# cvg/LightGlue

Measured on AMD Instinct MI355X. Metric: image-pairs/s at N=M=1024, 9 layers; match-index parity vs ref, higher is better.
Workload: dtype f16; 1 GPU; SuperPoint-dim 256-d descriptors, N=M=1024, 9 layers, pruning/early-stop OFF, batch=32 pairs per GPU, seeded random weights (recipe A), precision=f16x3 (split-f16 operands, 3 MFMAs per product, for every contraction incl. q k^T and P V; fp32 accumulate / residual / softmax); pairs_per_gpu=32, keypoints=1024, keypoints1=1024, descriptor_dim=256, parallelism=pair-sharded dp1, batches_in_flight=1

## Files before the change

lightglue_amd/csrc/lg_assign.hip:

```cpp
#include "lg_kernels.h"

namespace lg {

__device__ __forceinline__ float fexp(float x) { return __builtin_amdgcn_exp2f(x * 1.44269504088896340736f); }

__device__ __forceinline__ void lse_merge(float& m, float& s, float m2, float s2) {
    const float mn = fmaxf(m, m2);
    if (mn == -INFINITY) { m = mn; s = 0.f; return; }
    s = s * fexp(m - mn) + s2 * fexp(m2 - mn);
    m = mn;
}

constexpr int ART = 32;

__device__ __forceinline__ void lse_merge1(float& m, float& s, float m2, float s2) {
    const float e = (m == m2) ? 1.f : fexp(-fabsf(m - m2));
    const bool keep = m >= m2;
    s = keep ? __builtin_fmaf(s2, e, s) : __builtin_fmaf(s, e, s2);
    m = keep ? m : m2;
}

__global__ __launch_bounds__(256) void lse_sweep_kernel(AssignArgs a) {
    const int pair = blockIdx.y, tile = blockIdx.x, tid = threadIdx.x, lane = tid & 63, wave = tid >> 6;
    const int len0 = a.rs.len[2 * pair], len1 = a.rs.len[2 * pair + 1];
    const int r0 = tile * ART;
    if (r0 >= len0) return;
    const int rows = min(ART, len0 - r0);
    const int ntiles = a.rs.cap0 / ART;
    const float* simp = a.sim + ((long long)pair * a.rs.cap0 + r0) * a.rs.cap1;
    float* pm = a.cpm + ((long long)pair * ntiles + tile) * a.rs.cap1;
    float* ps = a.cps + ((long long)pair * ntiles + tile) * a.rs.cap1;
    __shared__ float shm[4][ART], shs[4][ART];
    for (int c0 = 0; c0 < len1; c0 += 1024) {
        const int c = c0 + tid * 4;
        const bool act = c < len1;
        const float* col = simp + (act ? c : 0);
        float cm[4] = {-INFINITY, -INFINITY, -INFINITY, -INFINITY}, cs[4] = {0.f, 0.f, 0.f, 0.f};
        f32x4 nxt = *reinterpret_cast<const f32x4*>(col);
#pragma unroll 1
        for (int r = 0; r < rows; ++r) {
            f32x4 v = nxt;
            nxt = *reinterpret_cast<const f32x4*>(col + (long long)min(r + 1, rows - 1) * a.rs.cap1);
#pragma unroll
            for (int i = 0; i < 4; ++i) if (!act || c + i >= len1) v[i] = -INFINITY;
            const float m = wave_allmax(fmaxf(fmaxf(v[0], v[1]), fmaxf(v[2], v[3])));
            float sum = 0.f;
            if (m != -INFINITY) sum = (fexp(v[0] - m) + fexp(v[1] - m)) + (fexp(v[2] - m) + fexp(v[3] - m));
            if (act) {
#pragma unroll
                for (int i = 0; i < 4; ++i) lse_merge1(cm[i], cs[i], v[i], v[i] == -INFINITY ? 0.f : 1.f);
            }
            sum = wave_allsum(sum);
            if (lane == 0) {
                if (c0 == 0) { shm[wave][r] = m; shs[wave][r] = sum; }
                else { float mo = shm[wave][r], so = shs[wave][r]; lse_merge1(mo, so, m, sum); shm[wave][r] = mo; shs[wave][r] = so; }
            }
        }
        if (act) {
            *reinterpret_cast<f32x4*>(pm + c) = f32x4{cm[0], cm[1], cm[2], cm[3]};
            *reinterpret_cast<f32x4*>(ps + c) = f32x4{cs[0], cs[1], cs[2], cs[3]};
        }
    }
    __syncthreads();
    if (tid < rows) {
        float m = shm[0][tid], s = shs[0][tid];
        for (int w = 1; w < 4; ++w) lse_merge1(m, s, shm[w][tid], shs[w][tid]);
        a.lse_r[(long long)pair * a.rs.cap0 + r0 + tid] = m + logf(s);
    }
}

__global__ __launch_bounds__(256) void col_lse_merge_kernel(AssignArgs a) {
    const int pair = blockIdx.y, lane = threadIdx.x & 63, wave = threadIdx.x >> 6, c = blockIdx.x * 64 + lane;
    const int len0 = a.rs.len[2 * pair], len1 = a.rs.len[2 * pair + 1];
    if (blockIdx.x * 64 >= len1) return;
    const int ntiles = a.rs.cap0 / ART, live = (len0 + ART - 1) / ART;
    const int cc = min(c, a.rs.cap1 - 1);
    const float* pm = a.cpm + (long long)pair * ntiles * a.rs.cap1 + cc;
    const float* ps = a.cps + (long long)pair * ntiles * a.rs.cap1 + cc;
    float m = -INFINITY, s = 0.f;
#pragma unroll 8
    for (int t = wave; t < live; t += 4) lse_merge1(m, s, pm[(long long)t * a.rs.cap1], ps[(long long)t * a.rs.cap1]);
    __shared__ float shm[4][64], shs[4][64];
    shm[wave][lane] = m; shs[wave][lane] = s;
    __syncthreads();
    if (wave == 0 && c < len1) {
#pragma unroll
        for (int w = 1; w < 4; ++w) lse_merge1(m, s, shm[w][lane], shs[w][lane]);
        a.lse_c[(long long)pair * a.rs.cap1 + c] = m + logf(s);
    }
}

__device__ __forceinline__ float score_of(float sim, float lr, float lc, float cert) {
    return ((sim - lr) + (sim - lc)) + cert;
}

__global__ __launch_bounds__(256) void argmax_sweep_kernel(AssignArgs a) {
    const int pair = blockIdx.y, tile = blockIdx.x, tid = threadIdx.x, lane = tid & 63, wave = tid >> 6;
    const int len0 = a.rs.len[2 * pair], len1 = a.rs.len[2 * pair + 1];
    const int r0 = tile * ART;
    if (r0 >= len0) return;
    const int rows = min(ART, len0 - r0);
    const int ntiles = a.rs.cap0 / ART;
    const float* simp = a.sim + ((long long)pair * a.rs.cap0 + r0) * a.rs.cap1;
    const float* lsec = a.lse_c + (long long)pair * a.rs.cap1;
    const float* ls1 = a.ls + seg_row_base(a.rs, 2 * pair + 1);
    const float* lser = a.lse_r + (long long)pair * a.rs.cap0 + r0;
    const float* ls0 = a.ls + seg_row_base(a.rs, 2 * pair) + r0;
    float* pv = a.cbv + ((long long)pair * ntiles + tile) * a.rs.cap1;
    int* pi = a.cbi + ((long long)pair * ntiles + tile) * a.rs.cap1;
    __shared__ float shb[4][ART]; __shared__ int shi[4][ART];
    for (int c0 = 0; c0 < len1; c0 += 1024) {
        const int c = c0 + tid * 4;
        const bool act = c < len1;
        const int cc = act ? c : 0;
        const float* col = simp + cc;
        const f32x4 lc = *reinterpret_cast<const f32x4*>(lsec + cc);
        const f32x4 l1 = *reinterpret_cast<const f32x4*>(ls1 + cc);
        float cb[4] = {-INFINITY, -INFINITY, -INFINITY, -INFINITY}; int ci[4] = {0, 0, 0, 0};
        f32x4 nxt = *reinterpret_cast<const f32x4*>(col);
#pragma unroll 1
        for (int r = 0; r < rows; ++r) {
// ... 133 lines not shown
    const int base0 = seg_row_base(a.rs, 2 * pair), base1 = seg_row_base(a.rs, 2 * pair + 1);
    float* out = a.log_assignment + (long long)pair * (a.n0 + 1) * (a.n1 + 1);
    if (len0 == 0 || len1 == 0) {
        if (r == a.rs.cap0 && tid == 0) out[(long long)a.n0 * (a.n1 + 1) + a.n1] = 0.f;
        return;
    }
    if (r == a.rs.cap0) {
        for (int c = tid; c < len1; c += 256) out[(long long)a.n0 * (a.n1 + 1) + a.ind[base1 + c]] = a.lsneg[base1 + c];
        if (tid == 0) out[(long long)a.n0 * (a.n1 + 1) + a.n1] = 0.f;
        return;
    }
    if (r >= len0) return;
    float* orow = out + (long long)a.ind[base0 + r] * (a.n1 + 1);
    const float* simr = a.sim + ((long long)pair * a.rs.cap0 + r) * a.rs.cap1;
    const float lr = a.lse_r[(long long)pair * a.rs.cap0 + r], l0 = a.ls[base0 + r];
    const float* lsec = a.lse_c + (long long)pair * a.rs.cap1;
    for (int c = tid; c < len1; c += 256) orow[a.ind[base1 + c]] = score_of(simr[c], lr, lsec[c], l0 + a.ls[base1 + c]);
    if (tid == 0) orow[a.n1] = a.lsneg[base0 + r];
}

hipError_t launch_assign(const AssignArgs& a, hipStream_t s) {
    const int B = a.rs.B;
    hipError_t e;
    if (!a.all_rows_live) {
    if (a.n0 > 0) {
        if ((e = hipMemsetAsync(a.m0, 0xFF, sizeof(int) * (size_t)B * a.n0, s)) != hipSuccess) return e;
        if ((e = hipMemsetAsync(a.s0, 0, sizeof(float) * (size_t)B * a.n0, s)) != hipSuccess) return e;
    }
    if (a.n1 > 0) {
        if ((e = hipMemsetAsync(a.m1, 0xFF, sizeof(int) * (size_t)B * a.n1, s)) != hipSuccess) return e;
        if ((e = hipMemsetAsync(a.s1, 0, sizeof(float) * (size_t)B * a.n1, s)) != hipSuccess) return e;
    }
    }
    hipLaunchKernelGGL(lse_sweep_kernel, dim3(a.rs.cap0 / ART, B), dim3(256), 0, s, a);
    hipLaunchKernelGGL(col_lse_merge_kernel, dim3(a.rs.cap1 / 64, B), dim3(256), 0, s, a);
    hipLaunchKernelGGL(argmax_sweep_kernel, dim3(a.rs.cap0 / ART, B), dim3(256), 0, s, a);
    hipLaunchKernelGGL(col_argmax_merge_kernel, dim3(a.rs.cap1 / 64, B), dim3(256), 0, s, a);
    hipLaunchKernelGGL(finalize_kernel, dim3((max(a.rs.cap0, a.rs.cap1) + 255) / 256, B), dim3(256), 0, s, a);
    if (a.log_assignment) {
        const long long total = (long long)B * (a.n0 + 1) * (a.n1 + 1);
        hipLaunchKernelGGL(fill_neg_inf_kernel, dim3(2048), dim3(256), 0, s, a.log_assignment, total);
        hipLaunchKernelGGL(log_assignment_kernel, dim3(a.rs.cap0 + 1, B), dim3(256), 0, s, a);
    }
    return hipGetLastError();
}

}
```

lightglue_amd/csrc/lg_engine.hip:

```cpp
#include <cmath>
#include <cstring>
#include <string>

#include "lg_engine.h"

using namespace lg;

namespace {

inline int round_up(int x, int m) { return (x + m - 1) / m * m; }
size_t attn_elem_bytes(int attn_prec) { return attn_prec == PREC_F32 ? 4 : attn_prec == PREC_F16X3 ? 4 : 2; }
int compact_chunks(int c0, int c1) { return (c0 > c1 ? c0 : c1) / compact_chunk_rows(); }
size_t cflags_bytes(int B, int c0, int c1) { return (size_t)2 * B * compact_chunks(c0, c1) * 4 + 256; }

}

namespace lg {

size_t workspace_layout(lg_engine* e, char* base, int B, int c0, int c1) {
    const size_t R = (size_t)B * (c0 + c1), as = attn_elem_bytes(e->attn_prec);
    const size_t per0 = (size_t)B * c0 * 4, per1 = (size_t)B * c1 * 4, tiles = (size_t)B * (c0 / 32) * c1 * 4;
    Arena ar{base};
    if (base) e->bufs.clear();
    auto take = [&](const char* name, auto*& member, size_t bytes) { ar.take(member, bytes); if (base) e->bufs[name] = {member, bytes}; };
// ... 60 lines not shown
void lg_engine_destroy(lg_engine* e) {
    if (!e) return;
    for (auto& sp : e->prof_pool) { (void)hipEventDestroy(sp.a); (void)hipEventDestroy(sp.b); }
    if (e->ws) (void)hipFree(e->ws);
    if (e->w_arena) (void)hipFree(e->w_arena);
    delete e;
}

static int check_envelope(long long B, long long n0, long long n1) {
    const long long c0 = (n0 + 127) / 128 * 128, c1 = (n1 + 127) / 128 * 128;
    if (n0 > LG_MAX_KEYPOINTS || n1 > LG_MAX_KEYPOINTS)
        return set_error(LG_ERR_INVALID, "more than LG_MAX_KEYPOINTS (8192) keypoints in one image");
    if (B * (c0 + c1) > LG_MAX_ROWS)
        return set_error(LG_ERR_INVALID, "batch * (cap0 + cap1) exceeds LG_MAX_ROWS (2^21 keypoint rows per forward): split the batch across calls");
    if (B * c0 * c1 > LG_MAX_SIM_ELEMS)
        return set_error(LG_ERR_INVALID, "batch * cap0 * cap1 exceeds LG_MAX_SIM_ELEMS (2^31 - 1 similarity entries per forward): split the batch across calls");
    return LG_OK;
}

int lg_engine_reserve(lg_engine* e, int32_t max_batch, int32_t max_n0, int32_t max_n1) {
    if (!e || max_batch < 1 || max_n0 < 0 || max_n1 < 0) return set_error(LG_ERR_INVALID, "bad argument");
    TRY(check_envelope(max_batch, max_n0, max_n1));
    return ensure_workspace(e, max_batch, max_n0, max_n1);
}

int lg_engine_set_option(lg_engine* e, const char* key, int32_t value) {
    if (!e || !key) return set_error(LG_ERR_INVALID, "null argument");
    if (std::strcmp(key, "fused_tail") == 0) { e->opt.fused_tail = value != 0; return LG_OK; }
    if (std::strcmp(key, "fused_next") == 0) { e->opt.fused_next = value != 0; return LG_OK; }
    if (std::strcmp(key, "fused_prep") == 0) { e->opt.fused_prep = value != 0; return LG_OK; }
    if (std::strcmp(key, "attn_dma") == 0) { e->opt.attn_dma = value != 0; return LG_OK; }
    if (std::strcmp(key, "adapt_gather") == 0) { e->opt.adapt_gather = value != 0; return LG_OK; }
    if (std::strcmp(key, "sim_planes") == 0) { e->opt.sim_planes = value != 0; return LG_OK; }
    if (std::strcmp(key, "sim_chunk") == 0) { if (value < 0 || value % 64) return set_error(LG_ERR_INVALID, "sim_chunk: 0 or a multiple of 64"); e->opt.sim_chunk = value; return LG_OK; }
    if (std::strcmp(key, "attn_rows") == 0) { if (value != 16 && value != 32 && value != 64) return set_error(LG_ERR_INVALID, "attn_rows must be 16, 32 or 64"); e->opt.attn_rows = value; e->opt.attn_auto_rows = false; return LG_OK; }
    if (std::strcmp(key, "tail_row_tiles") == 0) { if (value != 0 && value != 1 && value != 2 && value != 4) return set_error(LG_ERR_INVALID, "tail_row_tiles must be 0 (automatic), 1, 2 or 4"); e->opt.tail_row_tiles = value; return LG_OK; }
    if (std::strcmp(key, "profile_only") == 0) { e->prof_only = value; return LG_OK; }
    if (std::strcmp(key, "tail_timing") == 0) { e->opt.tail_timing = value; return LG_OK; }
    return set_error(LG_ERR_INVALID, std::string("unknown option '") + key + "'");
}

namespace {
int tail_row_tiles_for(int R) {
    int best = 4; long long best_cost = -1;
    const int shapes[3] = {4, 2, 1}; const long long cost[3] = {114, 69, 58};
    for (int i = 0; i < 3; ++i) {
        const long long wgs = R / (16 * shapes[i]), rounds = (wgs + 255) / 256, c = rounds * cost[i];
        if (best_cost < 0 || c < best_cost) { best = shapes[i]; best_cost = c; }
    }
    return best;
}

PairIndex pair_index(const lg_forward_io* io) { return indexed(io->flags) ? PairIndex{io->index0, io->index1, io->images0, io->images1} : PairIndex{}; }

int check_forward_io(const lg_engine* e, const lg_forward_io* io) {
    if (!e || !io) return set_error(LG_ERR_INVALID, "null argument");
    for (int side = 0; side < 2; ++side) {
        const SideFormat f = side_format(io->flags, side);
        if (!f.valid) return set_error(LG_ERR_INVALID, (io->flags & LG_FLAG_EXT) ? "LG_FLAG_DESC*_U8 and LG_FLAG_DESC*_F16 are both set on one side: a store has one format"
                                                                                 : "LG_FLAG_DESC*_F16 / LG_FLAG_DESC*_U8 / LG_FLAG_ROOTSIFT* need LG_FLAG_EXT");
        if (f.kind != DESC_F32 && (reinterpret_cast<uintptr_t>(side ? io->desc1 : io->desc0) & 15))
            return set_error(LG_ERR_INVALID, "LG_FLAG_DESC*_F16 / LG_FLAG_DESC*_U8: the descriptor pointer must be 16-byte aligned");
        if ((f.kind == DESC_U8 || f.rootsift) && e->cfg.input_dim % 4) return set_error(LG_ERR_INVALID, "LG_FLAG_DESC*_U8 / LG_FLAG_ROOTSIFT*: input_dim must be a multiple of 4");
        if (f.rootsift && e->cfg.input_dim > 256) return set_error(LG_ERR_INVALID, "LG_FLAG_ROOTSIFT0 / _ROOTSIFT1: input_dim must be at most 256 (one wave holds the row)");
    }
    const bool ext = (io->flags & LG_FLAG_EXT) != 0;
// ... 240 lines not shown
            {
                GemmArgs g = gemm_args(e, c, c.rs_act, e->X, D, e->MSG, D, D, 512, bw.f1, (size_t)i * 512 * 512, bw.b_f1 + (size_t)i * 512, 512, e->H1);
                PROFILED(PC_GEMM_FFN1, launch_gemm(prec, EPI_STORE, g, c.s));
            }
            if (plan.stops_at(step++)) return LG_OK;
            {
                LnGeluArgs ln{c.rs_act, e->H1, e->G, bw.ln_g + (size_t)i * 512, bw.ln_b + (size_t)i * 512, c.R};
                PROFILED(PC_LN_GELU, launch_ln_gelu(ln, c.s));
            }
            if (plan.stops_at(step++)) return LG_OK;
            {
                GemmArgs g = gemm_args(e, c, c.rs_act, e->G, 512, nullptr, 0, 512, 512, bw.f2, (size_t)i * D * 512, bw.b_f2 + (size_t)i * D, D, e->X);
                PROFILED(PC_GEMM_FFN2, launch_gemm(prec, EPI_RESID, g, c.s));
            }
            if (plan.stops_at(step++)) return LG_OK;
        }
        const AdaptMode mode = plan.after_layer(i);
        if (mode != AdaptMode::None) TRY(launch_adaptive_step(e, io, plan, c, i, mode));
    }
    stopped = false;
    return LG_OK;
}

int forward_assign(lg_engine* e, const lg_forward_io* io, const ForwardPlan& plan, const ForwardCtx& c) {
    const int prec = e->cfg.precision, n0 = io->n0, n1 = io->n1, D = 256;
    if (!plan.fused_tail) {
        RowDotArgs rd{};
        rd.rs = c.rs_all; rd.X = e->X; rd.w0 = e->w_match; rd.b0 = e->b_match; rd.out0 = e->LS; rd.act0 = 2;
        rd.layer_of_pair = e->FINAL_LAYER; rd.w_layer_stride = D; rd.ignore_active = 1;
        if (plan.wants_log_assignment) { rd.w1 = e->w_match; rd.b1 = e->b_match; rd.out1 = e->LSNEG; rd.act1 = 3; }
        PROFILED(PC_ROWDOT, launch_rowdot(rd, c.s));
    }
    if (!plan.final_proj_in_last_tail()) PROFILED(PC_GEMM_FINAL, launch_final_proj(prec, final_args(e, plan, c, true), c.s));
    TRY(prof_begin(e, PC_SIM, c.s));
    if (plan.sim_planes) {
        SimPlanesArgs sp{c.rs_all, reinterpret_cast<const f16_t*>(e->MD), (long long)c.R * 256, D, e->SIM, e->opt.sim_chunk};
        HIPCHK(launch_sim_planes(sp, c.s));
    } else {
        SimArgs sm{c.rs_all, e->MD, D, D, e->SIM};
        HIPCHK(launch_sim(prec, sm, c.s));
    }
    TRY(prof_end(e, c.s));
    AssignArgs as{};
    as.rs = c.rs_all; as.sim = e->SIM; as.ls = e->LS; as.lse_r = e->LSE_R; as.lse_c = e->LSE_C; as.max0 = e->MAX0; as.arg0 = e->ARG0;
    as.max1 = e->MAX1; as.arg1 = e->ARG1; as.cpm = e->CPM; as.cps = e->CPS; as.cbv = e->CBV; as.cbi = e->CBI; as.ind = e->IND; as.n0 = n0; as.n1 = n1; as.filter_threshold = (float)e->cfg.filter_threshold;
    as.m0 = io->matches0; as.m1 = io->matches1; as.s0 = io->scores0; as.s1 = io->scores1;
    as.matches = io->matches; as.mscores = io->match_scores; as.n_matches = io->n_matches; as.max_matches = n0 < n1 ? n0 : n1;
    as.log_assignment = io->log_assignment; as.lsneg = e->LSNEG;
    as.dbg = e->opt.tail_timing == 4 ? e->TAILDBG : nullptr;
    as.all_rows_live = plan.all_rows_live ? 1 : 0;
    PROFILED(PC_ASSIGN, launch_assign(as, c.s));
    HIPCHK(write_outputs(e, io, e->FINAL_LAYER, 0, c.range_flag, c.device_err, c.s));
    return LG_OK;
}
#undef PROFILED
}

int lg_engine_forward(lg_engine* e, const lg_forward_io* io, void* hip_stream) {
    TRY(check_forward_io(e, io));
    hipStream_t s = static_cast<hipStream_t>(hip_stream);
    if (io->n0 == 0 || io->n1 == 0) return forward_empty(e, io, s);
    TRY(ensure_workspace(e, io->batch, io->n0, io->n1));
    const ForwardPlan plan = plan_forward(e->cfg, e->attn_prec, e->opt, io->n0, io->n1, io->flags, io->num0 || io->num1, io->log_assignment != nullptr,
                                          launch_tail_supports_next(e->cfg.precision, e->attn_prec));
    const ForwardCtx c = forward_ctx(e, io, plan, s);
    bool stopped = false;
    TRY(forward_prepare(e, io, plan, c, stopped));
    if (stopped) return LG_OK;
    TRY(forward_layers(e, io, plan, c, stopped));
    if (stopped) return LG_OK;
    return forward_assign(e, io, plan, c);
}

}
```

lightglue_amd/csrc/lg_forward_plan.h:

```cpp
#pragma once
#include <cstdint>

#include "../../include/lightglue_amd.h"

namespace lg {

struct ForwardOptions {
    int fused_tail = 1, fused_next = 1, fused_prep = 1;
    bool adapt_gather = true;
    bool sim_planes = true;
    int sim_chunk = 0;
    bool attn_dma = true;
    int attn_rows = 32;
    bool attn_auto_rows = true;
    int tail_row_tiles = 0;
    int tail_timing = 0;
    int debug_stop = -1;
};

inline bool pruning_on(const lg_config& cfg, uint32_t io_flags) { return cfg.width_confidence > 0 && !(io_flags & LG_FLAG_NO_PRUNING); }
inline bool indexed(uint32_t io_flags) { return (io_flags & LG_FLAG_EXT) && (io_flags & LG_FLAG_INDEXED); }

enum : int { DESC_F32 = 0, DESC_F16 = 1, DESC_U8 = 2 };
struct SideFormat {
    int kind;
    bool rootsift;
    bool valid;
};
static_assert(LG_FLAG_DESC1_F16 == LG_FLAG_DESC0_F16 << 1 && LG_FLAG_DESC1_U8 == LG_FLAG_DESC0_U8 << 1 && LG_FLAG_ROOTSIFT1 == LG_FLAG_ROOTSIFT0 << 1, "side 1's flag = side 0's << 1");
inline SideFormat side_format(uint32_t io_flags, int side) {
    const bool f16 = io_flags & (LG_FLAG_DESC0_F16 << side), u8 = io_flags & (LG_FLAG_DESC0_U8 << side), root = io_flags & (LG_FLAG_ROOTSIFT0 << side);
    if (!(io_flags & LG_FLAG_EXT)) return {DESC_F32, false, !(f16 || u8 || root)};
    return {u8 ? DESC_U8 : f16 ? DESC_F16 : DESC_F32, root, !(u8 && f16)};
}

enum class ProjBy {
    PrevTail,
    Own,
    OwnFirst,
    OwnGather
};
enum class TailNext { None, NextProj, FinalProj };
enum class AdaptMode { None, StopOnly, PruneInPlace, PruneGather };
inline bool prunes(AdaptMode m) { return m == AdaptMode::PruneInPlace || m == AdaptMode::PruneGather; }

struct BlockPlan {
    ProjBy proj_by;
    TailNext tail_next;
    bool want_tok, prune_here, want_ls, want_lsneg;
    int first_step;
    int buf_set;
};

struct ForwardPlan {
    int n_layers, debug_stop;
    bool fused_tail;
    bool do_stop, do_prune;
    bool prune_possible;
    bool check_finite;
    bool fuse_prep;
    bool fuse_next;
    bool use_gather;
    bool sim_planes;
    bool split_qkv;
    bool all_rows_live;
    bool wants_log_assignment;

    bool stops_at(int step) const { return debug_stop >= 0 && step >= debug_stop; }
    int last_step() const { return 12 * n_layers; }

    AdaptMode after_layer(int layer) const {
        if (layer < 0 || layer + 1 >= n_layers) return AdaptMode::None;
        if (prune_possible) return use_gather ? AdaptMode::PruneGather : AdaptMode::PruneInPlace;
        return do_stop ? AdaptMode::StopOnly : AdaptMode::None;
    }

    TailNext tail_next(int layer, int blk) const {
        if (!fuse_next) return TailNext::None;
        const bool last = layer + 1 == n_layers;
        if (blk == 0 || (!last && !prune_possible)) return TailNext::NextProj;
        return last && !do_stop ? TailNext::FinalProj : TailNext::None;
    }

    BlockPlan block(int layer, int blk) const {
        BlockPlan b{};
        const bool first = layer == 0 && blk == 0, last = layer + 1 == n_layers;
        if (!first && tail_next(layer - (blk ^ 1), blk ^ 1) == TailNext::NextProj) b.proj_by = ProjBy::PrevTail;
        else if (first && fuse_prep) b.proj_by = ProjBy::OwnFirst;
        else if (blk == 0 && after_layer(layer - 1) == AdaptMode::PruneGather) b.proj_by = ProjBy::OwnGather;
        else b.proj_by = ProjBy::Own;
        b.tail_next = tail_next(layer, blk);
        if (blk == 1) {
            b.want_tok = !last && do_stop; b.prune_here = !last && prune_possible;
            b.want_ls = last || do_stop; b.want_lsneg = b.want_ls && wants_log_assignment;
        }
        b.first_step = 1 + 12 * layer + 6 * blk;
        b.buf_set = after_layer(0) == AdaptMode::PruneGather ? layer & 1 : 0;
        return b;
    }

    bool final_proj_in_last_tail() const { return tail_next(n_layers - 1, 1) == TailNext::FinalProj; }
};

inline ForwardPlan plan_forward(const lg_config& cfg, int attn_prec, const ForwardOptions& opt, int n0, int n1, uint32_t io_flags, bool has_counts,
                                bool wants_log_assignment, bool tail_supports_next) {
    ForwardPlan p{};
    p.n_layers = cfg.n_layers; p.debug_stop = opt.debug_stop; p.fused_tail = opt.fused_tail != 0; p.wants_log_assignment = wants_log_assignment;
    p.do_stop = cfg.depth_confidence > 0; p.do_prune = pruning_on(cfg, io_flags);
    p.prune_possible = p.do_prune && (n0 > cfg.pruning_min_kpts || n1 > cfg.pruning_min_kpts);
    p.check_finite = (io_flags & LG_FLAG_EXT) && (io_flags & LG_FLAG_CHECK_FINITE);
    const bool sift_store = (io_flags & LG_FLAG_EXT) && (io_flags & LG_SIFT_STORE_FLAGS);
    p.fuse_prep = opt.fused_prep && cfg.input_dim == 256 && opt.debug_stop < 0 && opt.tail_timing != 2 && !sift_store;
    p.fuse_next = opt.fused_next && opt.fused_tail && (opt.tail_timing == 0 || opt.tail_timing == 5 || opt.tail_timing == 6) &&
                  opt.debug_stop < 0 && tail_supports_next;
    p.use_gather = opt.adapt_gather && opt.fused_tail && opt.debug_stop < 0 && opt.tail_timing == 0;
    p.sim_planes = cfg.precision == LG_PREC_F16X3 && opt.sim_planes;
    p.split_qkv = attn_prec == LG_PREC_F16X3;
    p.all_rows_live = !p.do_prune && !has_counts && !indexed(io_flags);
    return p;
}

}
```

lightglue_amd/csrc/lg_kernels.h:

```cpp
#pragma once
#include <string>

#include "lg_common.h"

namespace lg {

int set_error(int code, const std::string& msg);
#define HIPCHK(expr)                                                                              \
    do {                                                                                          \
        hipError_t _e = (expr);                                                                   \
        if (_e != hipSuccess)                                                                     \
            return lg::set_error(LG_ERR_HIP, std::string(#expr) + ": " + hipGetErrorString(_e));  \
    } while (0)

template <class... KArgs, class... Args>
hipError_t launch_with_lds(void (*kern)(KArgs...), dim3 grid, dim3 threads, int smem, hipStream_t s, const Args&... args) {
    hipError_t e = hipFuncSetAttribute(reinterpret_cast<const void*>(kern), hipFuncAttributeMaxDynamicSharedMemorySize, smem);
    if (e != hipSuccess) return e;
    hipLaunchKernelGGL(kern, grid, threads, smem, s, args...);
    return hipGetLastError();
}

enum : int { EPI_STORE = 0, EPI_RESID = 1 };

struct GemmArgs {
    RowSpace rs;
    const float* A;  int lda;
    const float* A2; int lda2;
    int K1, K;
    const void* W;  const void* Wlo;
    const float* bias;
    int Nout;
    const int* layer_of_pair; long long w_layer_stride; long long b_layer_stride;
    float* out; int ldo; float out_scale;
    int R;
};
hipError_t launch_gemm(int prec, int epi, const GemmArgs& a, hipStream_t s);

struct SimArgs {
    RowSpace rs;
    const float* X; int ldx; int K;
    float* sim;
};
hipError_t launch_sim(int prec, const SimArgs& a, hipStream_t s);
struct SimPlanesArgs {
    RowSpace rs;
    const f16_t* md; long long plane; int K;
    float* sim;
    int chunk;
};
hipError_t launch_sim_planes(const SimPlanesArgs& a, hipStream_t s);

struct ProjArgs {
    RowSpace rs;
    const float* X;
    const void* W; const float* bias; int Nout;
    void* q; void* k; void* vt;
    long long plane;
    const float* cosb; const float* sinb;
    int n_qk_groups; int R;
    long long* dbg;
    int* range_flag;
};
hipError_t launch_proj(int prec, int attn_prec, const ProjArgs& a, hipStream_t s);
struct GatherArgs {
    const float* Xold; const float* cos_old; const float* sin_old;
    float* Xnew; float* cos_new; float* sin_new;
    const int* src;
    const int* len_old;
};
hipError_t launch_proj_gather(int prec, int attn_prec, const ProjArgs& a, const GatherArgs& g, hipStream_t s);

struct FinalArgs {
    RowSpace rs;
    const float* X;
    const void* W; const float* bias;
    const int* layer_of_pair; long long w_layer_bytes;
    float* out; float scale;
    int R;
    int planes;
    const float* X2; const int* xsel;
};
// ... 74 lines not shown
    int* prune0; int* prune1;
    int n0, n1;
    const int* len_orig;
    const float* conf; const float* mscore;
    float* X; float* cosb; float* sinb;
    int layer; float conf_thr; float depth_conf; float width_conf; int pruning_min_kpts;
    int do_stop, do_prune;
    int compact_chunks;
    int* compact_flags;
    int compact_epoch;
    int* compact_err;
    int* compact_ticket;
    int gather; int* src; int* xsel; int xnext;
};
hipError_t launch_adapt(const AdaptArgs& a, hipStream_t s);
int compact_chunk_rows();

struct AssignArgs {
    RowSpace rs;
    const float* sim;
    const float* ls;
    float* lse_r; float* lse_c;
    float* max0; int* arg0;
    float* max1; int* arg1;
    float* cpm; float* cps;
    float* cbv; int* cbi;
    const int* ind;
    int n0, n1;
    float filter_threshold;
    int* m0; int* m1; float* s0; float* s1;
    int* matches; float* mscores; int* n_matches; int max_matches;
    float* log_assignment; const float* lsneg;
    long long* dbg;
    int all_rows_live;
};
hipError_t launch_assign(const AssignArgs& a, hipStream_t s);

struct InitStateArgs {
    int B, n0, n1, L;
    const int* num0; const int* num1;
    int* len; int* len_orig; int* len_old; int* active; int* final_layer;
    int* prune0; int* prune1;
    int* range_flag; int* device_err; int* xsel;
    PairIndex px;
};
hipError_t launch_init_state(const InitStateArgs& a, hipStream_t s);
struct OutArgs {
    int B, n0, n1, L, kmax;
    const int* final_layer; int stop_const;
    int* stop;
    const int* m0; const int* m1; const float* s0; const float* s1; const int* matches; const int* n_matches;
    const int* prune0; const int* prune1; const int* num0; const int* num1;
    long long* m0_64; long long* m1_64; long long* matches_64; long long* stop_64; long long* prune0_64; long long* prune1_64;
    float* prune0_f; float* prune1_f;
    int* wire; long long wire_stride; int wire_prune;
    int* status; const int* range_flag; const int* device_err;
    PairIndex px;
};
hipError_t launch_write_outputs(const OutArgs& a, hipStream_t s);

}
```

lightglue_amd/csrc/lg_sim.hip:

```cpp
#include "lg_kernels.h"

namespace lg {

constexpr int SBM = 128, STHREADS = 512, SHALF = 2 * 32 * 512;

__global__ __launch_bounds__(STHREADS, 4) void sim_planes_kernel(SimPlanesArgs a) {
    typedef TagF16 Tag;
    extern __shared__ __attribute__((aligned(16))) char smem[];
    const int SCHUNK = a.chunk;
    const int strips = a.rs.cap0 / SBM, chunks = (a.rs.cap1 + SCHUNK - 1) / SCHUNK, per_pair = strips * chunks;
    const int v = xcd_remap(blockIdx.x, gridDim.x);
    const int pair = v / per_pair, rem = v - pair * per_pair;
    const int a0 = (rem / chunks) * SBM, b0 = (rem % chunks) * SCHUNK;
    const int len0 = a.rs.len[2 * pair], len1 = a.rs.len[2 * pair + 1];
    if (a0 >= len0 || b0 >= len1) return;
    const int nst = (min(len1 - b0, SCHUNK) + 63) >> 6;
    const int ntile = 2 * nst;
    const int tid = threadIdx.x, lane = tid & 63, wave = __builtin_amdgcn_readfirstlane(tid >> 6), lr = lane & 15, g = lane >> 4;
    const long long PL = a.plane;
    const f16_t* A = a.md + (seg_row_base(a.rs, 2 * pair) + a0) * 256LL;
    const f16_t* Bm = a.md + (seg_row_base(a.rs, 2 * pair + 1) + b0) * 256LL;

    uint32_t doff[4];
#pragma unroll
    for (int i = 0; i < 4; ++i) {
        const int rho = 2 * (4 * (wave & 3) + i) + (lane >> 5), sl = (lane & 31) ^ (rho & 15);
        doff[i] = (uint32_t)(((4 * (rho & 15) + (rho >> 4)) * 256 + sl * 8) * (int)sizeof(f16_t));
    }
    const f16_t* dbase = Bm + (wave >> 2) * PL;
    auto dma_tile = [&](int tile) {
        const f16_t* src = dbase + (64 * (tile >> 1) + 2 * (tile & 1)) * 256;
        char* dst = smem + (tile & 1) * SHALF + (wave >> 2) * (32 * 512) + (4 * (wave & 3)) * 1024;
#pragma unroll
        for (int i = 0; i < 4; ++i) lds_dma16_s(src, doff[i], dst + i * 1024);
    };
    dma_tile(0);

    u32x4 ah[8], al[8];
    {
        const f16_t* src = A + (16 * wave + lr) * 256 + 8 * g;
#pragma unroll
        for (int c = 0; c < 8; ++c) {
            ah[c] = *reinterpret_cast<const u32x4*>(src + 32 * c);
            al[c] = *reinterpret_cast<const u32x4*>(src + 32 * c + PL);
        }
    }
    int fo[4];
#pragma unroll
    for (int i = 0; i < 4; ++i) fo[i] = lr * 512 + (((i ^ (lr >> 2)) << 6) | ((g ^ (lr & 3)) << 4));

    f32x4 acc[4];
#pragma unroll
    for (int e = 0; e < 4; ++e) acc[e] = f32x4{0.f, 0.f, 0.f, 0.f};
    float* out = a.sim + ((long long)pair * a.rs.cap0 + a0 + 16 * wave + 4 * g) * a.rs.cap1 + b0 + 4 * lr;
    auto store_tile = [&](int T) {
#pragma unroll
        for (int r = 0; r < 4; ++r)
            *reinterpret_cast<f32x4*>(out + (long long)r * a.rs.cap1 + 64 * T) = f32x4{acc[0][r], acc[1][r], acc[2][r], acc[3][r]};
    };
    auto compute_half = [&](int h) {
        const char* base = smem + h * SHALF;
        u32x4 bh[2][2], bl[2][2];
        auto load_b = [&](int c, u32x4 (&hh)[2], u32x4 (&ll)[2]) {
#pragma unroll
            for (int nb = 0; nb < 2; ++nb) {
                const char* src = base + fo[c & 3] + (c >> 2) * 256 + nb * (16 * 512);
                hh[nb] = *reinterpret_cast<const u32x4*>(src);
                ll[nb] = *reinterpret_cast<const u32x4*>(src + 32 * 512);
            }
        };
        load_b(0, bh[0], bl[0]);
#pragma unroll
        for (int c = 0; c < 8; ++c) {
            if (c < 7) load_b(c + 1, bh[(c + 1) & 1], bl[(c + 1) & 1]);
            __builtin_amdgcn_sched_barrier(0);
#pragma unroll
            for (int nb = 0; nb < 2; ++nb) mma_chunk<Tag>(acc[2 * h + nb], al[c], bh[c & 1][nb]);
#pragma unroll
            for (int nb = 0; nb < 2; ++nb) mma_chunk<Tag>(acc[2 * h + nb], ah[c], bl[c & 1][nb]);
#pragma unroll
            for (int nb = 0; nb < 2; ++nb) mma_chunk<Tag>(acc[2 * h + nb], ah[c], bh[c & 1][nb]);
            __builtin_amdgcn_sched_barrier(0);
        }
    };
    for (int T = 0; T < nst; ++T) {
        wait_vmcnt0();
        asm volatile("" ::: "memory");
        __syncthreads();
        dma_tile(2 * T + 1);
        __builtin_amdgcn_sched_barrier(0);
        compute_half(0);
        wait_vmcnt0();
        asm volatile("" ::: "memory");
        __syncthreads();
        dma_tile(T + 1 < nst ? 2 * T + 2 : 2 * T);
        __builtin_amdgcn_sched_barrier(0);
        compute_half(1);
        store_tile(T);
#pragma unroll
        for (int e = 0; e < 4; ++e) acc[e] = f32x4{0.f, 0.f, 0.f, 0.f};
    }
    wait_vmcnt0();
    (void)ntile;
}

hipError_t launch_sim_planes(const SimPlanesArgs& a0, hipStream_t s) {
    SimPlanesArgs a = a0;
    if (a.rs.cap0 % SBM || a.rs.cap1 % 64 || a.K != 256 || !a.md || a.plane <= 0) return hipErrorInvalidValue;
    const int strips = a.rs.cap0 / SBM;
    int chunk = 512;
    while (chunk > 64 && (long long)strips * ((a.rs.cap1 + chunk - 1) / chunk) * a.rs.B < 512) chunk >>= 1;
    if (a.chunk <= 0) a.chunk = chunk;
    if (a.chunk % 64) return hipErrorInvalidValue;
    const int chunks = (a.rs.cap1 + a.chunk - 1) / a.chunk;
    hipLaunchKernelGGL(sim_planes_kernel, dim3(strips * chunks * a.rs.B), dim3(STHREADS), 2 * SHALF, s, a);
    return hipGetLastError();
}

}
```

Before: 4272 image-pairs/s.

## Fuse log-sum-exp partials into sim GEMM epilogue and merge rows/cols in one kernel

The similarity GEMM kernel now computes per-tile row and column log-sum-exp partials straight from its accumulators in registers. It writes them to the CPM/CPS buffers, so the separate lse_sweep pass that re-read the full sim matrix is skipped by default. The row and column merges are combined into one lse_merge_kernel, and the fallback sweep is rewritten in the same tiled form. The cost is extra reductions, LDS and barriers in the GEMM epilogue, which may hurt GEMM occupancy or overlap. The partial buffer layout also grows to hold row partials.

```diff
diff --git a/lightglue_amd/csrc/lg_assign.hip b/lightglue_amd/csrc/lg_assign.hip
--- a/lightglue_amd/csrc/lg_assign.hip
+++ b/lightglue_amd/csrc/lg_assign.hip
@@ -1,8 +1,7 @@
 #include "lg_kernels.h"
+#include "lg_lse_tile.h"
 
 namespace lg {
-
-__device__ __forceinline__ float fexp(float x) { return __builtin_amdgcn_exp2f(x * 1.44269504088896340736f); }
 
 __device__ __forceinline__ void lse_merge(float& m, float& s, float m2, float s2) {
     const float mn = fmaxf(m, m2);
@@ -13,80 +12,57 @@
 
 constexpr int ART = 32;
 
-__device__ __forceinline__ void lse_merge1(float& m, float& s, float m2, float s2) {
-    const float e = (m == m2) ? 1.f : fexp(-fabsf(m - m2));
-    const bool keep = m >= m2;
-    s = keep ? __builtin_fmaf(s2, e, s) : __builtin_fmaf(s, e, s2);
-    m = keep ? m : m2;
-}
-
-__global__ __launch_bounds__(256) void lse_sweep_kernel(AssignArgs a) {
-    const int pair = blockIdx.y, tile = blockIdx.x, tid = threadIdx.x, lane = tid & 63, wave = tid >> 6;
-    const int len0 = a.rs.len[2 * pair], len1 = a.rs.len[2 * pair + 1];
-    const int r0 = tile * ART;
-    if (r0 >= len0) return;
-    const int rows = min(ART, len0 - r0);
-    const int ntiles = a.rs.cap0 / ART;
-    const float* simp = a.sim + ((long long)pair * a.rs.cap0 + r0) * a.rs.cap1;
-    float* pm = a.cpm + ((long long)pair * ntiles + tile) * a.rs.cap1;
-    float* ps = a.cps + ((long long)pair * ntiles + tile) * a.rs.cap1;
-    __shared__ float shm[4][ART], shs[4][ART];
-    for (int c0 = 0; c0 < len1; c0 += 1024) {
-        const int c = c0 + tid * 4;
-        const bool act = c < len1;
-        const float* col = simp + (act ? c : 0);
-        float cm[4] = {-INFINITY, -INFINITY, -INFINITY, -INFINITY}, cs[4] = {0.f, 0.f, 0.f, 0.f};
-        f32x4 nxt = *reinterpret_cast<const f32x4*>(col);
-#pragma unroll 1
-        for (int r = 0; r < rows; ++r) {
-            f32x4 v = nxt;
-            nxt = *reinterpret_cast<const f32x4*>(col + (long long)min(r + 1, rows - 1) * a.rs.cap1);
-#pragma unroll
-            for (int i = 0; i < 4; ++i) if (!act || c + i >= len1) v[i] = -INFINITY;
-            const float m = wave_allmax(fmaxf(fmaxf(v[0], v[1]), fmaxf(v[2], v[3])));
-            float sum = 0.f;
-            if (m != -INFINITY) sum = (fexp(v[0] - m) + fexp(v[1] - m)) + (fexp(v[2] - m) + fexp(v[3] - m));
-            if (act) {
-#pragma unroll
-                for (int i = 0; i < 4; ++i) lse_merge1(cm[i], cs[i], v[i], v[i] == -INFINITY ? 0.f : 1.f);
-            }
-            sum = wave_allsum(sum);
-            if (lane == 0) {
-                if (c0 == 0) { shm[wave][r] = m; shs[wave][r] = sum; }
-                else { float mo = shm[wave][r], so = shs[wave][r]; lse_merge1(mo, so, m, sum); shm[wave][r] = mo; shs[wave][r] = so; }
-            }
-        }
-        if (act) {
-            *reinterpret_cast<f32x4*>(pm + c) = f32x4{cm[0], cm[1], cm[2], cm[3]};
-            *reinterpret_cast<f32x4*>(ps + c) = f32x4{cs[0], cs[1], cs[2], cs[3]};
-        }
-    }
-    __syncthreads();
-    if (tid < rows) {
-        float m = shm[0][tid], s = shs[0][tid];
-        for (int w = 1; w < 4; ++w) lse_merge1(m, s, shm[w][tid], shs[w][tid]);
-        a.lse_r[(long long)pair * a.rs.cap0 + r0 + tid] = m + logf(s);
-    }
-}
-
-__global__ __launch_bounds__(256) void col_lse_merge_kernel(AssignArgs a) {
-    const int pair = blockIdx.y, lane = threadIdx.x & 63, wave = threadIdx.x >> 6, c = blockIdx.x * 64 + lane;
-    const int len0 = a.rs.len[2 * pair], len1 = a.rs.len[2 * pair + 1];
-    if (blockIdx.x * 64 >= len1) return;
-    const int ntiles = a.rs.cap0 / ART, live = (len0 + ART - 1) / ART;
-    const int cc = min(c, a.rs.cap1 - 1);
-    const float* pm = a.cpm + (long long)pair * ntiles * a.rs.cap1 + cc;
-    const float* ps = a.cps + (long long)pair * ntiles * a.rs.cap1 + cc;
+constexpr int LSW_COLS = 256;
+__global__ __launch_bounds__(512) void lse_sweep_kernel(AssignArgs a) {
+    const int pair = blockIdx.y, tid = threadIdx.x, lane = tid & 63, wave = __builtin_amdgcn_readfirstlane(tid >> 6), lr = lane & 15, g = lane >> 4;
+    const int chunks = (a.rs.cap1 + LSW_COLS - 1) / LSW_COLS, strips = a.rs.cap0 / LSE_STRIP;
+    const int a0 = ((int)blockIdx.x / chunks) * LSE_STRIP, b0 = ((int)blockIdx.x % chunks) * LSW_COLS;
+    const int len0 = a.rs.len[2 * pair], len1 = a.rs.len[2 * pair + 1];
+    if (a0 >= len0 || b0 >= len1) return;
+    const int nst = (min(len1 - b0, LSW_COLS) + LSE_TILE - 1) / LSE_TILE;
+    __shared__ float lds[2 * LSE_LDS_FLOATS];
+    const int row0 = a0 + 16 * wave + 4 * g, col0 = b0 + 4 * lr;
+    const float* src = a.sim + ((long long)pair * a.rs.cap0 + row0) * a.rs.cap1 + col0;
+    const long long co = ((long long)pair * strips + a0 / LSE_STRIP) * a.rs.cap1 + b0;
+    const long long ro = lse_row_partials_offset(a.rs) + ((long long)pair * (a.rs.cap1 / LSE_TILE) + b0 / LSE_TILE) * a.rs.cap0;
+    auto load_tile = [&](int T, f32x4 (&x)[4]) {
+#pragma unroll
+        for (int r = 0; r < 4; ++r) x[r] = *reinterpret_cast<const f32x4*>(src + (long long)r * a.rs.cap1 + LSE_TILE * T);
+    };
+    f32x4 nxt[4];
+    load_tile(0, nxt);
+    for (int T = 0; T < nst; ++T) {
+        f32x4 acc[4];
+#pragma unroll
+        for (int e = 0; e < 4; ++e) acc[e] = f32x4{nxt[0][e], nxt[1][e], nxt[2][e], nxt[3][e]};
+        load_tile(min(T + 1, nst - 1), nxt);
+        lse_tile_partials(acc, row0, col0 + LSE_TILE * T, len0, len1, a.cpm + ro + (long long)T * a.rs.cap0, a.cps + ro + (long long)T * a.rs.cap0,
+                          lds + (T & 1) * LSE_LDS_FLOATS, wave, lr, g);
+        __syncthreads();
+        if (wave == (T & 7)) lse_col_flush(lds + (T & 1) * LSE_LDS_FLOATS, lane, a.cpm + co + LSE_TILE * T, a.cps + co + LSE_TILE * T);
+    }
+}
+
+__global__ __launch_bounds__(256) void lse_merge_kernel(AssignArgs a) {
+    const int pair = blockIdx.y, cols = blockIdx.z, lane = threadIdx.x & 63, wave = threadIdx.x >> 6, c = blockIdx.x * 64 + lane;
+    const int len0 = a.rs.len[2 * pair], len1 = a.rs.len[2 * pair + 1];
+    const int items = cols ? len1 : len0, cap = cols ? a.rs.cap1 : a.rs.cap0;
+    if ((int)blockIdx.x * 64 >= items) return;
+    const int nparts = cols ? a.rs.cap0 / LSE_STRIP : a.rs.cap1 / LSE_TILE, live = cols ? (len0 + LSE_STRIP - 1) / LSE_STRIP : (len1 + LSE_TILE - 1) / LSE_TILE;
+    const int cc = min(c, cap - 1);
+    const long long base = (cols ? 0 : lse_row_partials_offset(a.rs)) + (long long)pair * nparts * cap + cc;
+    const float* pm = a.cpm + base;
+    const float* ps = a.cps + base;
     float m = -INFINITY, s = 0.f;
 #pragma unroll 8
-    for (int t = wave; t < live; t += 4) lse_merge1(m, s, pm[(long long)t * a.rs.cap1], ps[(long long)t * a.rs.cap1]);
+    for (int t = wave; t < live; t += 4) lse_merge1(m, s, pm[(long long)t * cap], ps[(long long)t * cap]);
     __shared__ float shm[4][64], shs[4][64];
     shm[wave][lane] = m; shs[wave][lane] = s;
     __syncthreads();
-    if (wave == 0 && c < len1) {
+    if (wave == 0 && c < items) {
 #pragma unroll
         for (int w = 1; w < 4; ++w) lse_merge1(m, s, shm[w][lane], shs[w][lane]);
-        a.lse_c[(long long)pair * a.rs.cap1 + c] = m + logf(s);
+        (cols ? a.lse_c : a.lse_r)[(long long)pair * cap + c] = m + logf(s);
     }
 }
 
@@ -286,8 +262,8 @@
         if ((e = hipMemsetAsync(a.s1, 0, sizeof(float) * (size_t)B * a.n1, s)) != hipSuccess) return e;
     }
     }
-    hipLaunchKernelGGL(lse_sweep_kernel, dim3(a.rs.cap0 / ART, B), dim3(256), 0, s, a);
-    hipLaunchKernelGGL(col_lse_merge_kernel, dim3(a.rs.cap1 / 64, B), dim3(256), 0, s, a);
+    if (!a.lse_from_sim) hipLaunchKernelGGL(lse_sweep_kernel, dim3(a.rs.cap0 / LSE_STRIP * ((a.rs.cap1 + LSW_COLS - 1) / LSW_COLS), B), dim3(512), 0, s, a);
+    hipLaunchKernelGGL(lse_merge_kernel, dim3(max(a.rs.cap0, a.rs.cap1) / 64, B, 2), dim3(256), 0, s, a);
     hipLaunchKernelGGL(argmax_sweep_kernel, dim3(a.rs.cap0 / ART, B), dim3(256), 0, s, a);
     hipLaunchKernelGGL(col_argmax_merge_kernel, dim3(a.rs.cap1 / 64, B), dim3(256), 0, s, a);
     hipLaunchKernelGGL(finalize_kernel, dim3((max(a.rs.cap0, a.rs.cap1) + 255) / 256, B), dim3(256), 0, s, a);
diff --git a/lightglue_amd/csrc/lg_engine.hip b/lightglue_amd/csrc/lg_engine.hip
--- a/lightglue_amd/csrc/lg_engine.hip
+++ b/lightglue_amd/csrc/lg_engine.hip
@@ -116,6 +116,7 @@
     if (std::strcmp(key, "attn_dma") == 0) { e->opt.attn_dma = value != 0; return LG_OK; }
     if (std::strcmp(key, "adapt_gather") == 0) { e->opt.adapt_gather = value != 0; return LG_OK; }
     if (std::strcmp(key, "sim_planes") == 0) { e->opt.sim_planes = value != 0; return LG_OK; }
+    if (std::strcmp(key, "sim_lse") == 0) { e->opt.sim_lse = value != 0; return LG_OK; }
     if (std::strcmp(key, "sim_chunk") == 0) { if (value < 0 || value % 64) return set_error(LG_ERR_INVALID, "sim_chunk: 0 or a multiple of 64"); e->opt.sim_chunk = value; return LG_OK; }
     if (std::strcmp(key, "attn_rows") == 0) { if (value != 16 && value != 32 && value != 64) return set_error(LG_ERR_INVALID, "attn_rows must be 16, 32 or 64"); e->opt.attn_rows = value; e->opt.attn_auto_rows = false; return LG_OK; }
     if (std::strcmp(key, "tail_row_tiles") == 0) { if (value != 0 && value != 1 && value != 2 && value != 4) return set_error(LG_ERR_INVALID, "tail_row_tiles must be 0 (automatic), 1, 2 or 4"); e->opt.tail_row_tiles = value; return LG_OK; }
@@ -422,10 +423,16 @@
         PROFILED(PC_ROWDOT, launch_rowdot(rd, c.s));
     }
     if (!plan.final_proj_in_last_tail()) PROFILED(PC_GEMM_FINAL, launch_final_proj(prec, final_args(e, plan, c, true), c.s));
+    bool lse_from_sim = plan.sim_lse;
     TRY(prof_begin(e, PC_SIM, c.s));
     if (plan.sim_planes) {
-        SimPlanesArgs sp{c.rs_all, reinterpret_cast<const f16_t*>(e->MD), (long long)c.R * 256, D, e->SIM, e->opt.sim_chunk};
-        HIPCHK(launch_sim_planes(sp, c.s));
+        SimPlanesArgs sp{c.rs_all, reinterpret_cast<const f16_t*>(e->MD), (long long)c.R * 256, D, e->SIM, e->opt.sim_chunk, nullptr, nullptr};
+        if (lse_from_sim) { sp.cpm = e->CPM; sp.cps = e->CPS; }
+        if (lse_from_sim && launch_sim_planes(sp, c.s) != hipSuccess) {
+            (void)hipGetLastError();
+            lse_from_sim = false; sp.cpm = sp.cps = nullptr;
+        }
+        if (!lse_from_sim) HIPCHK(launch_sim_planes(sp, c.s));
     } else {
         SimArgs sm{c.rs_all, e->MD, D, D, e->SIM};
         HIPCHK(launch_sim(prec, sm, c.s));
@@ -438,7 +445,7 @@
     as.matches = io->matches; as.mscores = io->match_scores; as.n_matches = io->n_matches; as.max_matches = n0 < n1 ? n0 : n1;
     as.log_assignment = io->log_assignment; as.lsneg = e->LSNEG;
     as.dbg = e->opt.tail_timing == 4 ? e->TAILDBG : nullptr;
-    as.all_rows_live = plan.all_rows_live ? 1 : 0;
+    as.all_rows_live = plan.all_rows_live ? 1 : 0; as.lse_from_sim = lse_from_sim ? 1 : 0;
     PROFILED(PC_ASSIGN, launch_assign(as, c.s));
     HIPCHK(write_outputs(e, io, e->FINAL_LAYER, 0, c.range_flag, c.device_err, c.s));
     return LG_OK;
diff --git a/lightglue_amd/csrc/lg_forward_plan.h b/lightglue_amd/csrc/lg_forward_plan.h
--- a/lightglue_amd/csrc/lg_forward_plan.h
+++ b/lightglue_amd/csrc/lg_forward_plan.h
@@ -10,6 +10,7 @@
     bool adapt_gather = true;
     bool sim_planes = true;
     int sim_chunk = 0;
+    bool sim_lse = true;
     bool attn_dma = true;
     int attn_rows = 32;
     bool attn_auto_rows = true;
@@ -62,6 +63,7 @@
     bool fuse_next;
     bool use_gather;
     bool sim_planes;
+    bool sim_lse;
     bool split_qkv;
     bool all_rows_live;
     bool wants_log_assignment;
@@ -115,6 +117,7 @@
                   opt.debug_stop < 0 && tail_supports_next;
     p.use_gather = opt.adapt_gather && opt.fused_tail && opt.debug_stop < 0 && opt.tail_timing == 0;
     p.sim_planes = cfg.precision == LG_PREC_F16X3 && opt.sim_planes;
+    p.sim_lse = p.sim_planes && opt.sim_lse && !wants_log_assignment;
     p.split_qkv = attn_prec == LG_PREC_F16X3;
     p.all_rows_live = !p.do_prune && !has_counts && !indexed(io_flags);
     return p;
diff --git a/lightglue_amd/csrc/lg_kernels.h b/lightglue_amd/csrc/lg_kernels.h
--- a/lightglue_amd/csrc/lg_kernels.h
+++ b/lightglue_amd/csrc/lg_kernels.h
@@ -48,6 +48,7 @@
     const f16_t* md; long long plane; int K;
     float* sim;
     int chunk;
+    float* cpm; float* cps;
 };
 hipError_t launch_sim_planes(const SimPlanesArgs& a, hipStream_t s);
 
@@ -188,6 +189,7 @@
     int* matches; float* mscores; int* n_matches; int max_matches;
     float* log_assignment; const float* lsneg;
     long long* dbg;
+    int lse_from_sim;
     int all_rows_live;
 };
 hipError_t launch_assign(const AssignArgs& a, hipStream_t s);
diff --git a/lightglue_amd/csrc/lg_lse_tile.h b/lightglue_amd/csrc/lg_lse_tile.h
--- /dev/null
+++ b/lightglue_amd/csrc/lg_lse_tile.h
@@ -0,0 +1,58 @@
+#pragma once
+#include "lg_common.h"
+
+namespace lg {
+
+__device__ __forceinline__ float fexp(float x) { return __builtin_amdgcn_exp2f(x * 1.44269504088896340736f); }
+
+__device__ __forceinline__ void lse_merge1(float& m, float& s, float m2, float s2) {
+    const float e = (m == m2) ? 1.f : fexp(-fabsf(m - m2));
+    const bool keep = m >= m2;
+    s = keep ? __builtin_fmaf(s2, e, s) : __builtin_fmaf(s, e, s2);
+    m = keep ? m : m2;
+}
+
+constexpr int LSE_STRIP = 128, LSE_TILE = 64;
+constexpr int LSE_LDS_FLOATS = 2 * 8 * 64;
+constexpr int LSE_LDS_BYTES = 2 * LSE_LDS_FLOATS * 4;
+
+__host__ __device__ inline long long lse_row_partials_offset(const RowSpace& rs) { return (long long)rs.B * (rs.cap0 / LSE_STRIP) * rs.cap1; }
+
+__device__ __forceinline__ float row16_max(float x) {
+    x = vmax2(x, dpp_xor1(x)); x = vmax2(x, dpp_xor2(x)); x = vmax2(x, dpp_mov<0x141>(x)); return vmax2(x, dpp_mov<0x140>(x));
+}
+__device__ __forceinline__ float sum_exp4(float v0, float v1, float v2, float v3, float m) {
+    const float mm = m == -INFINITY ? 0.f : m;
+    return (fexp(v0 - mm) + fexp(v1 - mm)) + (fexp(v2 - mm) + fexp(v3 - mm));
+}
+__device__ __forceinline__ void lse_tile_partials(f32x4 (&acc)[4], int row0, int col0, int len0, int len1, float* rpm, float* rps, float* lds, int wave, int lr, int g) {
+#pragma unroll
+    for (int e = 0; e < 4; ++e)
+#pragma unroll
+        for (int r = 0; r < 4; ++r) acc[e][r] = (row0 + r < len0 && col0 + e < len1) ? acc[e][r] : -INFINITY;
+    float om = 0.f, os = 0.f;
+#pragma unroll
+    for (int r = 0; r < 4; ++r) {
+        const float m = row16_max(vmax2(vmax2(acc[0][r], acc[1][r]), vmax2(acc[2][r], acc[3][r])));
+        const float s = row16_sum(sum_exp4(acc[0][r], acc[1][r], acc[2][r], acc[3][r], m));
+        om = lr == r ? m : om; os = lr == r ? s : os;
+    }
+    if (lr < 4) { rpm[row0 + lr] = om; rps[row0 + lr] = os; }
+#pragma unroll
+    for (int e = 0; e < 4; ++e) {
+        const float m = xor32_max(xor16_max(vmax2(vmax2(acc[e][0], acc[e][1]), vmax2(acc[e][2], acc[e][3]))));
+        const float s = xor32_sum(xor16_sum(sum_exp4(acc[e][0], acc[e][1], acc[e][2], acc[e][3], m)));
+        om = g == e ? m : om; os = g == e ? s : os;
+    }
+    lds[wave * 64 + 4 * lr + g] = om;
+    lds[8 * 64 + wave * 64 + 4 * lr + g] = os;
+}
+
+__device__ __forceinline__ void lse_col_flush(const float* lds, int lane, float* cpm, float* cps) {
+    float m = lds[lane], s = lds[8 * 64 + lane];
+#pragma unroll
+    for (int w = 1; w < 8; ++w) lse_merge1(m, s, lds[w * 64 + lane], lds[8 * 64 + w * 64 + lane]);
+    cpm[lane] = m; cps[lane] = s;
+}
+
+}
diff --git a/lightglue_amd/csrc/lg_sim.hip b/lightglue_amd/csrc/lg_sim.hip
--- a/lightglue_amd/csrc/lg_sim.hip
+++ b/lightglue_amd/csrc/lg_sim.hip
@@ -1,9 +1,11 @@
 #include "lg_kernels.h"
+#include "lg_lse_tile.h"
 
 namespace lg {
 
 constexpr int SBM = 128, STHREADS = 512, SHALF = 2 * 32 * 512;
 
+template <bool LSE>
 __global__ __launch_bounds__(STHREADS, 4) void sim_planes_kernel(SimPlanesArgs a) {
     typedef TagF16 Tag;
     extern __shared__ __attribute__((aligned(16))) char smem[];
@@ -52,12 +54,21 @@
     f32x4 acc[4];
 #pragma unroll
     for (int e = 0; e < 4; ++e) acc[e] = f32x4{0.f, 0.f, 0.f, 0.f};
-    float* out = a.sim + ((long long)pair * a.rs.cap0 + a0 + 16 * wave + 4 * g) * a.rs.cap1 + b0 + 4 * lr;
+    float* out = a.sim + ((long long)pair * a.rs.cap0 + a0) * a.rs.cap1 + b0;
+    const uint32_t ooff = (uint32_t)(((16 * wave + 4 * g) * a.rs.cap1 + 4 * lr) * (int)sizeof(float));
     auto store_tile = [&](int T) {
 #pragma unroll
         for (int r = 0; r < 4; ++r)
-            *reinterpret_cast<f32x4*>(out + (long long)r * a.rs.cap1 + 64 * T) = f32x4{acc[0][r], acc[1][r], acc[2][r], acc[3][r]};
+            *reinterpret_cast<f32x4*>(reinterpret_cast<char*>(out + (long long)r * a.rs.cap1 + 64 * T) + ooff) = f32x4{acc[0][r], acc[1][r], acc[2][r], acc[3][r]};
     };
+    float* lse_lds = reinterpret_cast<float*>(smem + 2 * SHALF);
+    float *cpm = nullptr, *cps = nullptr, *rpm = nullptr, *rps = nullptr;
+    if constexpr (LSE) {
+        const long long co = ((long long)pair * strips + a0 / SBM) * a.rs.cap1 + b0;
+        const long long ro = lse_row_partials_offset(a.rs) + ((long long)pair * (a.rs.cap1 / LSE_TILE) + b0 / LSE_TILE) * a.rs.cap0;
+        cpm = a.cpm + co; cps = a.cps + co; rpm = a.cpm + ro; rps = a.cps + ro;
+    }
+    auto lane_now = []() { int l; asm volatile("v_mbcnt_lo_u32_b32 %0, -1, 0\n\tv_mbcnt_hi_u32_b32 %0, -1, %0" : "=v"(l)); return l; };
     auto compute_half = [&](int h) {
         const char* base = smem + h * SHALF;
         u32x4 bh[2][2], bl[2][2];
@@ -89,6 +100,9 @@
         __syncthreads();
         dma_tile(2 * T + 1);
         __builtin_amdgcn_sched_barrier(0);
+        if constexpr (LSE) {
+            if (T > 0 && wave == ((T - 1) & 7)) lse_col_flush(lse_lds + ((T - 1) & 1) * LSE_LDS_FLOATS, lane_now(), cpm + 64 * (T - 1), cps + 64 * (T - 1));
+        }
         compute_half(0);
         wait_vmcnt0();
         asm volatile("" ::: "memory");
@@ -97,10 +111,19 @@
         __builtin_amdgcn_sched_barrier(0);
         compute_half(1);
         store_tile(T);
+        if constexpr (LSE) {
+            const int t = lane_now(), lr2 = t & 15, g2 = t >> 4;
+            lse_tile_partials(acc, a0 + 16 * wave + 4 * g2, b0 + 64 * T + 4 * lr2, len0, len1, rpm + (long long)T * a.rs.cap0, rps + (long long)T * a.rs.cap0,
+                              lse_lds + (T & 1) * LSE_LDS_FLOATS, wave, lr2, g2);
+        }
 #pragma unroll
         for (int e = 0; e < 4; ++e) acc[e] = f32x4{0.f, 0.f, 0.f, 0.f};
     }
     wait_vmcnt0();
+    if constexpr (LSE) {
+        __syncthreads();
+        if (wave == ((nst - 1) & 7)) lse_col_flush(lse_lds + ((nst - 1) & 1) * LSE_LDS_FLOATS, lane, cpm + 64 * (nst - 1), cps + 64 * (nst - 1));
+    }
     (void)ntile;
 }
 
@@ -113,7 +136,9 @@
     if (a.chunk <= 0) a.chunk = chunk;
     if (a.chunk % 64) return hipErrorInvalidValue;
     const int chunks = (a.rs.cap1 + a.chunk - 1) / a.chunk;
-    hipLaunchKernelGGL(sim_planes_kernel, dim3(strips * chunks * a.rs.B), dim3(STHREADS), 2 * SHALF, s, a);
+    static_assert(SBM == LSE_STRIP, "a workgroup's rows are one strip of the log-sum-exp partials");
+    if (a.cpm) return launch_with_lds(sim_planes_kernel<true>, dim3(strips * chunks * a.rs.B), dim3(STHREADS), 2 * SHALF + LSE_LDS_BYTES, s, a);
+    hipLaunchKernelGGL(sim_planes_kernel<false>, dim3(strips * chunks * a.rs.B), dim3(STHREADS), 2 * SHALF, s, a);
     return hipGetLastError();
 }
 
```

Result: no change. 4277 image-pairs/s (median of 3 runs) (+0.1%).
